# JohnLCaron/electionguard-remote

Hardware: AMD Instinct MI355X
Metric: ballots verified+tallied/sec (node, 4096-bit group) (higher is better)
Workload: dtype u32xu32->u64 (radix-2^29 limbs)

## Files before the change

electionguard-remote_amd/csrc/eg_capi.hip:

```cpp
#include <hip/hip_runtime.h>

#include <algorithm>
#pragma clang diagnostic ignored "-Wunused-result"
#pragma clang diagnostic ignored "-Wunused-value"
#include <cstdio>
#include <cstdlib>
#include <cstring>
#include <deque>
#include <functional>
#include <array>
#include <atomic>
#include <chrono>
#include <condition_variable>
#include <map>
#include <memory>
#include <mutex>
#include <thread>
#include <string>
#include <vector>

#include "../../include/eg_hip.h"
#include "../../include/eg_hip_manifest.h"
#include "../../include/eg_hip_codes.h"
#include "../../include/eg_hip_contestdata.h"
// ... 113 lines not shown
  W_IN0, W_IN1, W_EXP, W_OUT, W_E0, W_E1, W_E2, W_E3, W_JOBS, W_SCR, W_TMP, W_FLAGS, W_SCAL,
  W_BE0, W_BE1, W_BE2, W_OK0, W_OK1, W_OFF, W_H0, W_H1, W_H2, W_H3, W_H4, W_H5, W_H6, W_H7, W_H8, W_EB0, W_EB1, W_EB2, W_EA2, W_YA, W_YB, W_RZ, W_CRF, W_CAST, W_ANY, W_GATHER, W_KBE, W_STAGE, W_NSLOT
};

struct eg_ctx {
  int device = 0;
  hipStream_t stream = nullptr;
  std::mutex mu;
  MontConsts h{};
  MontConsts* d = nullptr;
  uint8_t p_be[512], q_be[32], g_be[512];
  uint8_t* d_q = nullptr;
  uint8_t* d_qbar = nullptr;
  eg_fixed_base* gtab = nullptr;
  eg_fixed_base* Ktab = nullptr;
  uint32_t* d_gcomb = nullptr;
  uint32_t hash_fmt = EG_HASH_FIXED_WIDTH;
  uint32_t resp_plus = 0;
  uint32_t pre_order = EG_PREIMAGE_MESSAGE_FIRST;
  DevBuf ws[W_NSLOT];
  bool timing = false;
  std::vector<ProfRec> prof;
  uint64_t* d_clk = nullptr;
  size_t clk_used = 0;
  uint32_t clk_used_last = 0, clk_dropped_last = 0;
  uint8_t K_be[512];
  struct KeyTabs {
    std::array<uint8_t, 512> K;
    eg_fixed_base* fb = nullptr;
    eg_fixed_base* ct = nullptr;
    uint8_t* d_K = nullptr;
  };
  std::vector<KeyTabs> keys;
  std::map<std::string, DevBuf> cache;
  std::map<std::string, SchedBuf> sched;
  uint32_t use_comb = 1;
  uint32_t ct_encrypt = 0;
  uint32_t ct_pow = 0;
  std::atomic<uint32_t> ct_pow_submit{0};
  int ct_window = kCtEncWindow;
  eg_fixed_base* g_ct = nullptr;
  uint32_t ct_rows = 4;
  uint32_t sel_rows = 4;
  uint32_t sel_blocks = 3;
  size_t pow_slots = 0;
  uint32_t pow_wps = 3;
  double prof_clock_ghz = 0;
  std::vector<std::pair<std::array<uint8_t, 512>, eg_fixed_base*>> share_keys;
  std::shared_ptr<struct Coalescer> co;
  std::mutex co_mu;
  bool co_closed = false;
  hipStream_t copy = nullptr;
  hipEvent_t up_ev[2] = {nullptr, nullptr}, done_ev[2] = {nullptr, nullptr};
  void* comm = nullptr;
  int comm_world = 1, comm_rank = 0;
  bool comm_failed = false;
  std::string comm_fail_msg;
  Pow16Consts* lat = nullptr;
  size_t lat_jobs = 0;
  PowWaveConsts* latw = nullptr;
  size_t latw_jobs = 0;
  size_t wave_max = 0;
  bool wave_split = true;
  size_t r2l_max = 0;
  size_t w8_max = 0;
  int co_zc = 2;
  bool fb_lds = false;
  int test_fail_jobs = 0;
};

static int ws_get(eg_ctx* c, Slot s, size_t bytes, void** out) {
  DevBuf& b = c->ws[s];
  if (b.bytes < bytes) {
    if (b.ptr) HIPCHK(hipFree(b.ptr));
    b.ptr = nullptr;
    b.bytes = 0;
    size_t want = std::max(bytes, (size_t)4096);
    hipError_t e = hipMalloc(&b.ptr, want);
    if (e != hipSuccess) return fail(EG_ERR_NOMEM, "hipMalloc workspace " + std::to_string(want) + " B failed");
    b.bytes = want;
  }
  *out = b.ptr;
  return EG_OK;
}

#define LAUNCH_F(c, K, grid, ...)                                                              \
  do {                                                                                        \
    if ((c)->h.friendly)                                                                      \
      hipLaunchKernelGGL(K<true>, grid, dim3(kBlock), 0, (c)->stream, __VA_ARGS__);            \
    else                                                                                      \
      hipLaunchKernelGGL(K<false>, grid, dim3(kBlock), 0, (c)->stream, __VA_ARGS__);           \
  } while (0)

static inline unsigned grid_for(size_t groups) { return (unsigned)((groups + kGroupsPerBlock - 1) / kGroupsPerBlock); }
static inline size_t padded_groups(size_t groups) { return (size_t)grid_for(groups) * kGroupsPerBlock; }
static inline unsigned cgrid(size_t n) { return (unsigned)((n + 255) / 256); }

static bool aligned16(std::initializer_list<const void*> ps) {
  for (const void* p : ps)
    if ((uintptr_t)p & 15) return false;
  return true;
}

struct StreamOps {
  eg_ctx* c;
  int alloc(size_t bytes, void** out) const { return ws_get(c, W_STAGE, bytes, out); }
  int h2d(void* dst, const void* src, size_t bytes) const {
    HIPCHK(hipMemcpyAsync(dst, src, bytes, hipMemcpyHostToDevice, c->stream));
    return EG_OK;
  }
  int d2h(void* dst, const void* src, size_t bytes) const {
    HIPCHK(hipMemcpyAsync(dst, src, bytes, hipMemcpyDeviceToHost, c->stream));
    return EG_OK;
  }
  int sync() const {
    HIPCHK(hipStreamSynchronize(c->stream));
    return EG_OK;
  }
};
struct Stage : egstage::Stage<StreamOps> {
  Stage(eg_ctx* c, bool host, size_t n, size_t chunk) : egstage::Stage<StreamOps>(StreamOps{c}, host, n, chunk) {}
};

static int launch_import(eg_ctx* c, const uint8_t* d_be, size_t n, uint32_t* d_out, uint8_t* d_ltp) {
  if (!n) return EG_OK;
  LAUNCH_F(c, k_import, dim3(grid_for(n)), c->d, d_be, (uint32_t)n, d_out, d_ltp);
  HIPCHK(hipGetLastError());
  return EG_OK;
}
static int launch_export(eg_ctx* c, const uint32_t* d_in, size_t n, uint8_t* d_be) {
  if (!n) return EG_OK;
  LAUNCH_F(c, k_export, dim3(grid_for(n)), c->d, d_in, (uint32_t)n, d_be);
  HIPCHK(hipGetLastError());
  return EG_OK;
}

static std::vector<uint32_t> pow_schedule(const MontConsts& H, const PowShape& S, const FbTab& f0, const FbTab& f1,
                                          MMCount* mm) {
  std::vector<uint32_t> v;
  MMCount n;
  auto op = [&](PowOp k, uint32_t arg = 0) {
    v.push_back(pow_op(k, arg));
    if (k == OP_SQR) n.sqr += 1;
    else if (k != OP_END && k <= kOpMulLast) n.mul += 1;
  };
// ... 203 lines not shown
    uint32_t* scr = scratch;
    if (!scr) {
      const int rc = ws_get(c, W_SCR, padded_groups(nj) * per + padded_groups(nt) * per1 + padded_groups(nt2) * per2,
                            (void**)&scr);
      if (rc) return rc;
    }
    PowPart P0{S, sched, d_jobs + off * kJobWords, (uint32_t)nj, grid_for(nj), scr,
               yout ? yout + off * (kCombH - 1) * kW : nullptr, ygat, rout ? rout + off * 2 * kW : nullptr, ctab};
    PowPart P1{}, P2{};
    if (nt) {
      P1 = PowPart{tail->S, sched_tail, tail->jobs, (uint32_t)nt, grid_for(nt),
                   scr + padded_groups(nj) * per / 4, tail->yout, tail->ygat, tail->rout, tail->ctab};
    }
    if (nt2) {
      P2 = PowPart{tail2->S, sched_tail2, tail2->jobs, (uint32_t)nt2, grid_for(nt2),
                   scr + (padded_groups(nj) * per + padded_groups(nt) * per1) / 4, tail2->yout, tail2->ygat,
                   tail2->rout, tail2->ctab};
    }
    const dim3 grid(P0.nblocks + P1.nblocks + P2.nblocks);
    ProfRec* pr = nullptr;
    uint64_t* clk = nullptr;
    if (c->timing) {
      c->prof.push_back(ProfRec{nullptr, nullptr,
                                (mm_job.mul + mm_job.sqr) * (double)nj + (mm_tail.mul + mm_tail.sqr) * (double)nt +
                                    (mm_tail2.mul + mm_tail2.sqr) * (double)nt2,
                                mm_job.sqr * (double)nj + mm_tail.sqr * (double)nt + mm_tail2.sqr * (double)nt2});
      pr = &c->prof.back();
      HIPCHK(hipEventCreate(&pr->a));
      HIPCHK(hipEventCreate(&pr->b));
      if (c->d_clk && c->clk_used + grid.x <= kClockRecs) {
        clk = c->d_clk + 2 * c->clk_used;
        c->clk_used += grid.x;
      }
      HIPCHK(hipEventRecord(pr->a, c->stream));
    }
    if (c->h.friendly) {
      if (ct) hipLaunchKernelGGL((k_pow<true, true>), grid, dim3(kBlock), 0, c->stream, c->d, P0, P1, P2, d_elems, d_scal, d_out, f0, f1, clk);
      else hipLaunchKernelGGL((k_pow<true, false>), grid, dim3(kBlock), 0, c->stream, c->d, P0, P1, P2, d_elems, d_scal, d_out, f0, f1, clk);
    } else {
      if (ct) hipLaunchKernelGGL((k_pow<false, true>), grid, dim3(kBlock), 0, c->stream, c->d, P0, P1, P2, d_elems, d_scal, d_out, f0, f1, clk);
      else hipLaunchKernelGGL((k_pow<false, false>), grid, dim3(kBlock), 0, c->stream, c->d, P0, P1, P2, d_elems, d_scal, d_out, f0, f1, clk);
    }
    HIPCHK(hipGetLastError());
    if (pr) HIPCHK(hipEventRecord(pr->b, c->stream));
    off += nj;
  } while (off < njobs);
  return EG_OK;
}

template <class Pass>
static int prod_tree(eg_ctx* c, size_t groups, size_t len, size_t stride, uint32_t* d_out, Pass pass) {
  if (!groups) return EG_OK;
  if (len == 0) return fail(EG_ERR_ARG, "empty product");
  const uint32_t chunk = len > 32 ? 8u : 32u;
  const size_t maxpart = groups * ((len + chunk - 1) / chunk);
  uint32_t* tmp = nullptr;
  int rc = ws_get(c, W_TMP, std::max<size_t>(1, maxpart) * kW * 4 * 2, (void**)&tmp);
  if (rc) return rc;
  uint32_t* ping[2] = {tmp, tmp + maxpart * kW};
  size_t cur_len = len, cur_stride = stride;
  const uint32_t* src = nullptr;
  int pi = 0;
  while (true) {
    const uint32_t nchunk = (uint32_t)((cur_len + chunk - 1) / chunk);
    const bool last = nchunk == 1;
    uint32_t* dst = last ? d_out : ping[pi];
    pass(src, (uint32_t)cur_len, (uint32_t)cur_stride, last ? (uint32_t)cur_len : chunk, nchunk, dst, last);
    HIPCHK(hipGetLastError());
    if (last) break;
    src = dst;
    cur_len = nchunk;
    cur_stride = 1;
    pi ^= 1;
  }
  return EG_OK;
}

static int run_prod(eg_ctx* c, const uint32_t* d_in, GroupMap gm, size_t groups, size_t len, size_t stride,
                    uint32_t* d_out, const uint8_t* mask = nullptr) {
  return prod_tree(c, groups, len, stride, d_out,
                   [&](const uint32_t* src, uint32_t n, uint32_t st, uint32_t ch, uint32_t nchunk, uint32_t* dst, bool) {
                     LAUNCH_F(c, k_prod, dim3(grid_for(groups * nchunk)), c->d, src ? src : d_in,
                              src ? GroupMap{1, 1, 0, 0, n} : gm, (uint32_t)groups, n, st, ch, nchunk, dst,
                              src ? nullptr : mask);
                   });
}

static int run_prod_tab(eg_ctx* c, const uint32_t* d_in, const uint32_t* tab, size_t period, size_t period_stride,
                        size_t groups, size_t len, size_t stride, uint32_t* d_out, const uint32_t* otab,
                        size_t ostride, const uint8_t* mask = nullptr) {
  return prod_tree(c, groups, len, stride, d_out,
                   [&](const uint32_t* src, uint32_t n, uint32_t st, uint32_t ch, uint32_t nchunk, uint32_t* dst, bool last) {
                     LAUNCH_F(c, k_prod_tab, dim3(grid_for(groups * nchunk)), c->d, src ? src : d_in,
                              src ? nullptr : tab, (uint32_t)period, src ? n : (uint32_t)period_stride,
                              (uint32_t)groups, n, st, ch, nchunk, dst, last ? otab : nullptr, (uint32_t)ostride,
                              src ? nullptr : mask);
                   });
}

static int build_fb(eg_ctx* c, const uint32_t* d_base_mont, int wbits, eg_fixed_base* fb) {
  const int nwin = (256 + wbits - 1) / wbits;
  const size_t entries = (size_t)nwin << wbits;
  HIPCHK(hipMalloc(&fb->d_tab, entries * kW * 4));
  fb->wbits = wbits;
  fb->nwin = nwin;
  uint32_t* P = nullptr;
  const int npow = nwin * wbits;
  HIPCHK(hipMalloc(&P, (size_t)npow * kW * 4));
  LAUNCH_F(c, k_sqr_chain, dim3(1), c->d, d_base_mont, (uint32_t)npow, P);
  HIPCHK(hipGetLastError());
  for (int k = 0; k < nwin; ++k) {
    uint32_t* row = fb->d_tab + ((size_t)k << wbits) * kW;
    HIPCHK(hipMemcpyAsync(row, c->d->one, kW * 4, hipMemcpyDeviceToDevice, c->stream));
    for (int a = 0; a < wbits; ++a)
      HIPCHK(hipMemcpyAsync(row + ((size_t)1 << a) * kW, P + (size_t)(k * wbits + a) * kW, kW * 4,
                            hipMemcpyDeviceToDevice, c->stream));
  }
  for (int a = 1; a < wbits; ++a) {
    const size_t njobs = (size_t)nwin * (((size_t)1 << a) - 1);
    LAUNCH_F(c, k_fb_level, dim3(grid_for(njobs)), c->d, fb->d_tab,
                       (uint32_t)wbits, (uint32_t)nwin, (uint32_t)a);
    HIPCHK(hipGetLastError());
  }
  HIPCHK(hipStreamSynchronize(c->stream));
  HIPCHK(hipFree(P));
  return EG_OK;
}

static int import_one(eg_ctx* c, const uint8_t be[512], uint32_t** d_mont_out) {
  uint8_t* d_be = nullptr;
  uint32_t* d_m = nullptr;
  HIPCHK(hipMalloc(&d_be, 512));
  HIPCHK(hipMalloc(&d_m, kW * 4));
  HIPCHK(hipMemcpyAsync(d_be, be, 512, hipMemcpyHostToDevice, c->stream));
  int rc = launch_import(c, d_be, 1, d_m, nullptr);
  if (rc) return rc;
  HIPCHK(hipStreamSynchronize(c->stream));
  HIPCHK(hipFree(d_be));
  *d_mont_out = d_m;
  return EG_OK;
}

static int fb_create_locked(eg_ctx* c, const uint8_t base_be[512], int wbits, eg_fixed_base** out) {
  if (wbits < 4 || wbits > 22)
    return fail(EG_ERR_ARG, "window_bits must be in [4, 22]");
  uint32_t* d_m = nullptr;
  int rc = import_one(c, base_be, &d_m);
  if (rc) return rc;
  auto* fb = new eg_fixed_base();
// ... 39 lines not shown
  unit[0] = 1;
  words_to_elem(unit, c->h.unit);
  for (int i = 0; i < 128; ++i) c->h.pw[i] = p[i];
  uint32_t inv = 1;
  for (int i = 0; i < 6; ++i) inv *= 2u - p[0] * inv;
  c->h.n0 = (0u - inv) & kMask;
  c->h.friendly = c->h.n0 == 1 ? 1u : 0u;
  c->h.mask = kMask;
  {
    const char* lp = getenv("EG_LATENCY_POW");
    const std::string mode = lp ? lp : "";
    std::string err;
    if (mode != "0" && pow16_consts_create(p.data(), r2.data(), r.data(), c->h.n0, c->h.friendly, &c->lat, &err) == 0)
      c->lat_jobs = pow16_round_jobs(device) / 2;
    if (mode != "0" && mode != "16" &&
        powwave_consts_create(p.data(), r2.data(), r.data(), c->h.n0, c->h.friendly, &c->latw, &err) == 0) {
      int cus = 0;
      if (hipDeviceGetAttribute(&cus, hipDeviceAttributeMultiprocessorCount, device) == hipSuccess) {
        c->latw_jobs = (size_t)cus * 4;
        c->r2l_max = (size_t)cus;
        c->w8_max = (size_t)cus;
      }
      if (const char* w8 = getenv("EG_WAVE_W8")) c->w8_max = (size_t)std::max(0L, atol(w8));
      if (const char* rl = getenv("EG_WAVE_R2L")) c->r2l_max = (size_t)std::max(0L, atol(rl));
      if (const char* zc = getenv("EG_COALESCE_ZC")) {
        const std::string z = zc;
        c->co_zc = z == "in" ? 1 : z == "out" ? 2 : z == "inout" ? 3 : 0;
      }
      c->wave_max = c->latw_jobs;
      if (const char* wm = getenv("EG_WAVE_MAX")) c->wave_max = (size_t)std::max(0L, atol(wm));
      if (const char* ws = getenv("EG_WAVE_SPLIT")) c->wave_split = ws[0] != '0';
    }
  }
  {
    const Big q = be_to_words(q_be, 32);
    int64_t br = 0;
    for (int i = 0; i < 8; ++i) {
      br += -(int64_t)q[i];
      c->h.qc[i] = (uint32_t)br;
      br >>= 32;
    }
    c->h.qc_bits = 0;
    for (int b = 255; b >= 0; --b)
      if ((c->h.qc[b >> 5] >> (b & 31)) & 1u) { c->h.qc_bits = (uint32_t)b + 1; break; }
  }
  if (const char* nc = getenv("EG_NO_COMB")) c->use_comb = (nc[0] == '1') ? 0u : 1u;
  if (const char* cr = getenv("EG_CT_ROWS")) c->ct_rows = (cr[0] == '5') ? 0u : 4u;
  if (const char* sc = getenv("EG_SEL_COMB")) {
    c->sel_rows = (sc[0] == '5') ? 0u : 4u;
    c->sel_blocks = (sc[0] == '5') ? 2u : (sc[1] == '2' ? 2u : (sc[1] == '4' ? 4u : 3u));
  }
  if (const char* tf = getenv("EG_TEST_FAIL_JOBS")) c->test_fail_jobs = atoi(tf);
  if (const char* fl = getenv("EG_FB_LDS")) c->fb_lds = fl[0] == '1';
  if (const char* cw = getenv("EG_CT_WINDOW")) c->ct_window = std::max(4, std::min((int)kCtMaxWindow, atoi(cw)));
  {
    int cus = 0, per_cu = 0;
    const char* ts = getenv("EG_TAIL_SPLIT");
    if (!(ts && ts[0] == '0') && hipDeviceGetAttribute(&cus, hipDeviceAttributeMultiprocessorCount, device) == hipSuccess &&
        hipOccupancyMaxActiveBlocksPerMultiprocessor(&per_cu, k_pow<true, false>, kBlock, 0) == hipSuccess && per_cu > 0) {
      c->pow_slots = (size_t)cus * (size_t)per_cu;
      c->pow_wps = (uint32_t)std::max(1, per_cu * (kBlock / 64) / 4);
    }
  }
  hipError_t e = hipStreamCreateWithFlags(&c->stream, hipStreamNonBlocking);
  if (e != hipSuccess) {
    delete c;
    return fail(EG_ERR_HIP, std::string("hipStreamCreate: ") + hipGetErrorString(e));
  }
  auto setup = [&]() -> int {
    HIPCHK(hipMalloc(&c->d, sizeof(MontConsts)));
    HIPCHK(hipMemcpy(c->d, &c->h, sizeof(MontConsts), hipMemcpyHostToDevice));
    HIPCHK(hipMalloc(&c->d_q, 32));
    HIPCHK(hipMemcpy(c->d_q, q_be, 32, hipMemcpyHostToDevice));
    HIPCHK(hipMalloc(&c->d_qbar, 32));
    std::lock_guard<std::mutex> lk(c->mu);
    return fb_create_locked(c, g_be, 8, &c->gtab);
  };
  const int rc = setup();
  if (rc) {
    const std::string msg = g_err;
    eg_ctx_destroy(c);
    return fail(rc, msg);
  }
  *out = c;
  return EG_OK;
}

extern "C" int eg_fixed_base_destroy(eg_fixed_base* fb) {
  if (!fb) return EG_OK;
  while (fb->queued.load(std::memory_order_acquire) > 0) std::this_thread::sleep_for(std::chrono::microseconds(20));
  if (fb->d_tab) hipFree(fb->d_tab);
  eg_fixed_base_destroy(fb->ct);
  delete fb;
  return EG_OK;
}

static int ct_table_locked(eg_ctx* c, eg_fixed_base* fb, FbTab* out) {
  if (fb->wbits <= (int)kCtMaxWindow) {
    *out = fb->tab();
    return EG_OK;
  }
  if (!fb->ct) {
    const int rc = fb_create_locked(c, fb->base.data(), kCtEncWindow, &fb->ct);
    if (rc) return rc;
  }
  *out = fb->ct->tab();
  return EG_OK;
}

static void coalescer_stop(eg_ctx* c);
static int comm_destroy_locked(eg_ctx* c);

extern "C" int eg_ctx_destroy(eg_ctx* c) {
  if (!c) return EG_OK;
  coalescer_stop(c);
  hipSetDevice(c->device);
  hipStreamSynchronize(c->stream);
  comm_destroy_locked(c);
  eg_fixed_base_destroy(c->gtab);
  for (auto& k : c->keys) {
    eg_fixed_base_destroy(k.fb);
    eg_fixed_base_destroy(k.ct);
    if (k.d_K) hipFree(k.d_K);
  }
  eg_fixed_base_destroy(c->g_ct);
  for (auto& kv : c->share_keys) eg_fixed_base_destroy(kv.second);
  for (auto& b : c->ws)
    if (b.ptr) hipFree(b.ptr);
  for (auto& kv : c->cache)
    if (kv.second.ptr) hipFree(kv.second.ptr);
  for (auto& kv : c->sched) hipFree(const_cast<uint32_t*>(kv.second.ptr));
  for (auto& r : c->prof) {
    if (r.a) hipEventDestroy(r.a);
    if (r.b) hipEventDestroy(r.b);
  }
  if (c->d_clk) hipFree(c->d_clk);
  pow16_consts_destroy(c->lat);
  powwave_consts_destroy(c->latw);
  if (c->d) hipFree(c->d);
  if (c->d_q) hipFree(c->d_q);
  if (c->d_qbar) hipFree(c->d_qbar);
  if (c->d_gcomb) hipFree(c->d_gcomb);
  if (c->copy) {
    hipStreamSynchronize(c->copy);
    hipStreamDestroy(c->copy);
  }
  for (int i = 0; i < 2; ++i) {
    if (c->up_ev[i]) hipEventDestroy(c->up_ev[i]);
    if (c->done_ev[i]) hipEventDestroy(c->done_ev[i]);
  }
  if (c->stream) hipStreamDestroy(c->stream);
  delete c;
  return EG_OK;
}

extern "C" int eg_ctx_sync(eg_ctx* c) {
  if (!c) return fail(EG_ERR_ARG, "null ctx");
  HIPCHK(hipSetDevice(c->device));
  HIPCHK(hipStreamSynchronize(c->stream));
  return EG_OK;
}

extern "C" eg_fixed_base* eg_ctx_g_table(eg_ctx* c) { return c ? c->gtab : nullptr; }

extern "C" int eg_ctx_set_hash_format(eg_ctx* c, int format) {
  if (!c) return fail(EG_ERR_ARG, "null ctx");
  if (format != EG_HASH_FIXED_WIDTH && format != EG_HASH_MINIMAL) return fail(EG_ERR_ARG, "unknown hash format");
  std::lock_guard<std::mutex> lk(c->mu);
  c->hash_fmt = (uint32_t)format;
  return EG_OK;
}

extern "C" int eg_ctx_set_proof_format(eg_ctx* c, int response, int preimage) {
  if (!c) return fail(EG_ERR_ARG, "null ctx");
  if (response != EG_RESPONSE_MINUS && response != EG_RESPONSE_PLUS) return fail(EG_ERR_ARG, "unknown response convention");
  if (preimage < EG_PREIMAGE_MESSAGE_FIRST || preimage > EG_PREIMAGE_WITH_KEY)
    return fail(EG_ERR_ARG, "unknown pre-image order");
  std::lock_guard<std::mutex> lk(c->mu);
  c->resp_plus = response == EG_RESPONSE_PLUS ? 1u : 0u;
  c->pre_order = (uint32_t)preimage;
  return EG_OK;
}

extern "C" int eg_fixed_base_create(eg_ctx* c, const uint8_t base_be[512], int wbits, eg_fixed_base** out) {
  if (!c || !base_be || !out) return fail(EG_ERR_ARG, "null argument");
  std::lock_guard<std::mutex> lk(c->mu);
  HIPCHK(hipSetDevice(c->device));
  return fb_create_locked(c, base_be, wbits, out);
}

struct Locked {
  std::lock_guard<std::mutex> lk;
  explicit Locked(eg_ctx* c) : lk(c->mu) { hipSetDevice(c->device); }
};

static int upload(eg_ctx* c, Slot s, const void* h, size_t bytes, void** d) {
  int rc = ws_get(c, s, bytes, d);
  if (rc) return rc;
  HIPCHK(hipMemcpyAsync(*d, h, bytes, hipMemcpyHostToDevice, c->stream));
// ... 356 lines not shown
```

electionguard-remote_amd/csrc/eg_capi_ballot.inc:

```

static int upload_job_table(eg_ctx* c, const std::vector<uint32_t>& host, DevBuf* out) {
  DevBuf b;
  b.bytes = std::max<size_t>(4, host.size() * 4);
  if (c->test_fail_jobs > 0 && --c->test_fail_jobs == 0)
    return fail(EG_ERR_NOMEM, "hipMalloc job table failed (EG_TEST_FAIL_JOBS)");
  if (hipMalloc(&b.ptr, b.bytes) != hipSuccess)
    return fail(EG_ERR_NOMEM, "hipMalloc job table " + std::to_string(b.bytes) + " B failed");
  const hipError_t e = hipMemcpy(b.ptr, host.data(), host.size() * 4, hipMemcpyHostToDevice);
  if (e != hipSuccess) {
    hipFree(b.ptr);
    return fail(EG_ERR_HIP, std::string("hipMemcpy job table: ") + hipGetErrorString(e));
  }
  *out = b;
  return EG_OK;
}

static int cache_bound(eg_ctx* c) {
  if (c->cache.size() < 64) return EG_OK;
  HIPCHK(hipStreamSynchronize(c->stream));
  for (auto& kv : c->cache) HIPCHK(hipFree(kv.second.ptr));
  c->cache.clear();
  return EG_OK;
}

// ... 235 lines not shown
    std::vector<uint32_t> t;
    for (uint32_t k : C.members)
      for (uint32_t comp = 0; comp < 2; ++comp) t.push_back(M.first[k] * 2 + comp);
    return t;
  });
  L.add("out" + C.tag, &T.out[ci], [&C]() {
    std::vector<uint32_t> t;
    for (uint32_t k : C.members)
      for (uint32_t comp = 0; comp < 2; ++comp) t.push_back(k * 2 + comp);
    return t;
  });
}

static int contest_aggregates(eg_ctx* c, const ManShape& M, const ContestTabs& T, size_t nbc, const uint32_t* elems,
                              uint32_t* agg) {
  if (M.uniform)
    return run_prod(c, elems, GroupMap{2, (uint32_t)M.nc, 1, 2 * M.uspc, (uint32_t)(2 * M.nsel)}, nbc * M.nc * 2,
                    M.uspc, 2, agg);
  for (size_t ci = 0; ci < M.cls.size(); ++ci) {
    const size_t period = M.cls[ci].n * 2;
    const int rc = run_prod_tab(c, elems, T.in[ci], period, 2 * M.nsel, nbc * period, M.cls[ci].spc, 2, agg,
                                T.out[ci], 2 * M.nc);
    if (rc) return rc;
  }
  return EG_OK;
}
static void contest_scalars(eg_ctx* c, const ManShape& M, const ContestTabs& T, uint8_t* sc, size_t ncn, uint8_t* negL,
                            uint8_t* okc) {
  if (M.uniform)
    hipLaunchKernelGGL(k_scalar_prep, dim3(cgrid(ncn)), dim3(256), 0, c->stream, c->d_q, sc, (uint32_t)ncn, 2u, 0u,
                       M.ulimit, negL, okc, c->resp_plus, 0x1u);
  else
    hipLaunchKernelGGL(k_scalar_prep_tab, dim3(cgrid(ncn)), dim3(256), 0, c->stream, c->d_q, sc, (uint32_t)ncn, 2u, 0u,
                       T.limit, (uint32_t)M.nc, negL, okc, c->resp_plus, 0x1u);
}
static void contest_flags(eg_ctx* c, const ManShape& M, const ContestTabs& T, const uint8_t* ltp, size_t ncn,
                          uint8_t* crf) {
  if (M.uniform)
    hipLaunchKernelGGL(k_contest_flags, dim3(cgrid(ncn * 2)), dim3(256), 0, c->stream, ltp, (uint32_t)ncn, M.uspc,
                       crf);
  else
    hipLaunchKernelGGL(k_contest_flags_seg, dim3(cgrid(ncn * 2)), dim3(256), 0, c->stream, ltp, (uint32_t)ncn,
                       (uint32_t)M.nc, (uint32_t)M.nsel, T.first, T.spc, crf);
}
static void nonce_sums(eg_ctx* c, const ManShape& M, const ContestTabs& T, const uint8_t* sc, size_t ncn,
                       uint8_t* rsum) {
  if (M.uniform)
    hipLaunchKernelGGL(k_enc_rsum, dim3(cgrid(ncn)), dim3(256), 0, c->stream, c->d_q, sc, (uint32_t)ncn, M.uspc, rsum);
  else
    hipLaunchKernelGGL(k_enc_rsum_seg, dim3(cgrid(ncn)), dim3(256), 0, c->stream, c->d_q, sc, (uint32_t)ncn,
                       (uint32_t)M.nc, (uint32_t)M.nsel, T.first, T.spc, rsum);
}
static int chunk_tally(eg_ctx* c, const ManShape& M, const ContestTabs& T, size_t nbc, const uint32_t* elems,
                       uint32_t* out, const uint8_t* d_cast) {
  if (M.uniform)
    return run_prod(c, elems, GroupMap{2, M.uspc - M.uph, 1, 2, 2 * M.uspc}, M.nreal * 2, nbc, M.nsel * 2, out, d_cast);
  return run_prod_tab(c, elems, T.tally, M.nreal * 2, 0, M.nreal * 2, nbc, M.nsel * 2, out, nullptr, 0, d_cast);
}

struct VerifyLayout {
  size_t ns, ncn, off_c, off_neg, off_negL;
  VerifyLayout(const ManShape& M, size_t nbc)
      : ns(nbc * M.nsel), ncn(nbc * M.nc), off_c(ns * 4), off_neg(off_c + ncn * 2), off_negL(off_neg + ns) {}
};
static std::vector<uint32_t> verify_sel_jobs(const VerifyLayout& V, bool beta) {
  auto J = new_jobs(V.ns);
  for (size_t i = 0; i < V.ns; ++i) {
    uint32_t* x = &J[i * kJobWords];
    const uint32_t c0 = (uint32_t)(i * 4), v0 = c0 + 1, c1 = c0 + 2, v1 = c0 + 3, e = beta ? 1u : 0u;
    x[0] = (uint32_t)(i * 2) + e; x[1] = c0; x[2] = c1; x[3] = c0 + e; x[4] = c1 + e; x[5] = v0; x[7] = v1;
    if (beta) x[8] = (uint32_t)(V.off_neg + i);
  }
  return J;
}
static std::vector<uint32_t> verify_contest_jobs(const ManShape& M, const ManShape::Class& C, const VerifyLayout& V,
                                                 size_t nbc, bool b) {
  auto J = new_jobs(nbc * C.n);
  for (size_t bi = 0; bi < nbc; ++bi)
    for (size_t mi = 0; mi < C.n; ++mi) {
      const uint32_t k = M.member(C, mi), e = b ? 1u : 0u;
      const size_t j = bi * M.nc + k;
      uint32_t* x = &J[(bi * C.n + mi) * kJobWords];
      const uint32_t cc = (uint32_t)(V.off_c + j * 2);
      x[0] = (uint32_t)(V.ns * 2 + j * 2) + e; x[1] = cc; x[3] = (uint32_t)(V.ns * 4 + j * 2) + e; x[5] = cc + 1;
      if (b) x[6] = (uint32_t)(V.off_negL + j);
      x[2] = (uint32_t)(bi * M.nsel + M.first_of(k));
    }
  return J;
}

struct Pop {
  PowShape S;
  const uint32_t* jobs;
  size_t n;
  const uint32_t* ygat;
  Pop part(size_t off, size_t cnt) const { return Pop{S, jobs + off * kJobWords, cnt, ygat}; }
  PowTail tail() const {
    PowTail T{};
    T.S = S; T.jobs = jobs; T.njobs = n; T.ygat = ygat;
    return T;
  }
};
struct PowLaunch {
  Pop main;
  std::vector<Pop> tails;
};
struct VerifyPlan {
  size_t xb = 0;
  std::vector<Pop> l2;
  std::vector<PowLaunch> later;
// ... 103 lines not shown
    if ((rc = ws_get(c, W_YA, ns * (kCombH - 1) * kW * 4, (void**)&YA))) return rc;
    if ((rc = ws_get(c, W_YB, ns * (kCombH - 1) * kW * 4, (void**)&YB))) return rc;
  }
  if ((rc = ws_get(c, W_RZ, ns * 4 * kW * 4, (void**)&RZ))) return rc;
  const uint32_t srows = c->sel_rows, sblocks = c->sel_blocks;
  PowShape SA{};
  SA.has_base = 1; SA.nout = 2; SA.nfb[0] = 1; SA.nfb[1] = 1; SA.exp_bytes = 32; SA.comb = 1; SA.resid = 1;
  SA.rows = srows; SA.blocks = sblocks; SA.tab[0][0] = 0; SA.tab[1][0] = 0;
  PowShape SB{};
  SB.has_base = 1; SB.nout = 2; SB.nfb[0] = 1; SB.nfb[1] = 2; SB.exp_bytes = 32; SB.comb = 1; SB.resid = 1;
  SB.rows = srows; SB.blocks = sblocks; SB.tab[0][0] = 1; SB.tab[1][0] = 1; SB.tab[1][1] = 0;
  std::vector<Pop> pa, pb;
  for (size_t ci = 0; ci < ncls; ++ci) {
    const uint32_t gather = gat ? M.cls[ci].spc : 0u;
    const size_t n = nbc * M.cls[ci].n;
    PowShape SCA{};
    SCA.has_base = 1; SCA.nout = 1; SCA.nfb[0] = 1; SCA.exp_bytes = 32; SCA.tab[0][0] = 0;
    SCA.comb = gat ? 1u : 0u; SCA.gather = gather;
    PowShape SCB{};
    SCB.has_base = 1; SCB.nout = 1; SCB.nfb[0] = 2; SCB.exp_bytes = 32; SCB.tab[0][0] = 1; SCB.tab[0][1] = 0;
    SCB.comb = gat ? 1u : 0u; SCB.gather = gather;
    pa.push_back(Pop{SCA, jCA[ci], n, YA});
    pb.push_back(Pop{SCB, jCB[ci], n, YB});
  }
  const VerifyPlan P = plan_pow_launches(c, M, ns, ncn, pa, pb);
  const size_t xb = P.xb;
  auto launch = [&](const PowShape& S, const uint32_t* jobs, size_t n, uint32_t* yout, const uint32_t* ygat,
                    uint32_t* rout, const std::vector<PowTail>& tl) {
    return launch_pow(c, S, jobs, n, E, SC, COMM, G, K, yout, ygat, tl.size() > 0 ? &tl[0] : nullptr, rout, false,
                      nullptr, nullptr, tl.size() > 1 ? &tl[1] : nullptr);
  };
  auto tails_of = [](const std::vector<Pop>& pops) {
    std::vector<PowTail> tl;
    for (const Pop& p : pops) tl.push_back(p.tail());
    return tl;
  };
  {
    PowTail H{};
    H.S = SB; H.jobs = jB; H.njobs = xb; H.yout = YB; H.rout = RZ + ns * 2 * kW;
    if ((rc = launch(SA, jA, ns, YA, nullptr, RZ, {H}))) return rc;
  }
  if ((rc = launch(SB, jB + xb * kJobWords, ns - xb, gat ? YB + xb * (kCombH - 1) * kW : nullptr, nullptr,
                   RZ + (ns + xb) * 2 * kW, tails_of(P.l2))))
    return rc;
  LAUNCH_F(c, k_resid_check, dim3(grid_for(ns)), c->d, RZ, (uint32_t)ns, LTP, 2u);
  LAUNCH_F(c, k_resid_check, dim3(grid_for(ns)), c->d, RZ + ns * 2 * kW, (uint32_t)ns, LTP + 1, 2u);
  HIPCHK(hipGetLastError());
  uint8_t* CRF = nullptr;
  if ((rc = ws_get(c, W_CRF, ncn * 2, (void**)&CRF))) return rc;
  contest_flags(c, M, T, LTP, ncn, CRF);
  HIPCHK(hipGetLastError());
  for (const PowLaunch& l : P.later)
    if ((rc = launch(l.main.S, l.main.jobs, l.main.n, nullptr, l.main.ygat, nullptr, tails_of(l.tails)))) return rc;
  if ((rc = launch_export(c, COMM, ns * 4 + ncn * 2, COMM_BE))) return rc;
  if ((rc = launch_export(c, CP, ncn * 2, CP_BE))) return rc;
  if ((rc = launch_hash(c, (uint32_t)ns,
                        preimage(c, {HashSrc{cts, 512, 1024}, HashSrc{cts + 512, 512, 1024}},
                                 {HashSrc{COMM_BE, 512, 2048}, HashSrc{COMM_BE + 512, 512, 2048},
                                  HashSrc{COMM_BE + 1024, 512, 2048}, HashSrc{COMM_BE + 1536, 512, 2048}},
                                 key_src(c)),
                        d_rproof, 4, 0, 2, OKR, LTP, 2, d_ok_sel, nullptr)))
    return rc;
  const uint8_t* CC_BE = COMM_BE + ns * 4 * 512;
  if ((rc = launch_hash(c, (uint32_t)ncn,
                        preimage(c, {HashSrc{CP_BE, 512, 1024}, HashSrc{CP_BE + 512, 512, 1024}},
                                 {HashSrc{CC_BE, 512, 1024}, HashSrc{CC_BE + 512, 512, 1024}}, key_src(c)),
                        d_cproof, 2, 0, kNone, OKC, CRF, 2, d_ok_con, nullptr)))
    return rc;
  if (tally) {
    uint32_t* TP = first ? tally : tally + nreal * 2 * kW;
    if ((rc = chunk_tally(c, M, T, nbc, E, TP, d_cast))) return rc;
    if (!first) {
      LAUNCH_F(c, k_mul, dim3(grid_for(nreal * 2)), c->d, tally, 1u, TP, 1u, (uint32_t)(nreal * 2), tally, 1u);
      HIPCHK(hipGetLastError());
    }
  }
  return EG_OK;
}

static int use_key_locked(eg_ctx* c, const uint8_t* K_be) {
  for (size_t i = 0; i < c->keys.size(); ++i)
    if (std::memcmp(c->keys[i].K.data(), K_be, 512) == 0) {
      key_front(c, i);
      return EG_OK;
    }
  const int wb = c->Ktab ? c->Ktab->wbits : c->gtab->wbits;
  return set_key_locked(c, K_be, wb, false);
}

static void ones_be(uint8_t* out, size_t n) {
  std::memset(out, 0, n * 512);
  for (size_t i = 0; i < n; ++i) out[i * 512 + 511] = 1;
}

static int verify_dev_locked(eg_ctx* c, const ManShape& M, const uint8_t* qbar_be, size_t nb, const uint8_t* d_cts,
                             const uint8_t* d_rproof, const uint8_t* d_cproof, const uint8_t* d_cast,
                             uint8_t* d_ok_sel, uint8_t* d_ok_con, uint8_t* d_tally_be) {
  int rc;
  const size_t nc = M.nc, nsel = M.nsel, nreal = M.nreal;
  if (!nb) {
    if (d_tally_be) {
      std::vector<uint8_t> one(nreal * 2 * 512);
      ones_be(one.data(), nreal * 2);
      HIPCHK(hipMemcpyAsync(d_tally_be, one.data(), one.size(), hipMemcpyHostToDevice, c->stream));
      HIPCHK(hipStreamSynchronize(c->stream));
    }
    return EG_OK;
  }
  if (!c->Ktab) return fail(EG_ERR_STATE, "election key not set (eg_set_election_key)");
  HIPCHK(hipMemcpyAsync(c->d_qbar, qbar_be, 32, hipMemcpyHostToDevice, c->stream));
  uint32_t* tally = nullptr;
  if (d_tally_be && (rc = ws_get(c, W_E2, nreal * 2 * 2 * kW * 4, (void**)&tally))) return rc;
  const size_t chunk = ballot_chunk(nsel);
  for (size_t b0 = 0; b0 < nb; b0 += chunk) {
    const size_t nbc = std::min(chunk, nb - b0);
    if ((rc = verify_chunk_locked(c, M, nbc, d_cts + b0 * nsel * 1024, d_rproof + b0 * nsel * 128,
                                  d_cproof + b0 * nc * 64, d_cast ? d_cast + b0 : nullptr, d_ok_sel + b0 * nsel,
                                  d_ok_con + b0 * nc, tally, b0 == 0)))
      return rc;
  }
  return d_tally_be ? launch_export(c, tally, nreal * 2, d_tally_be) : EG_OK;
}

static int ensure_copy_stream(eg_ctx* c) {
  if (c->copy) return EG_OK;
  HIPCHK(hipStreamCreateWithFlags(&c->copy, hipStreamNonBlocking));
  for (int i = 0; i < 2; ++i) {
    HIPCHK(hipEventCreateWithFlags(&c->up_ev[i], hipEventDisableTiming));
// ... 537 lines not shown
```

electionguard-remote_amd/csrc/eg_kernels.hpp:

```cpp
#pragma once
#include "eg_bignum.hpp"
#include "eg_sha256.hpp"

namespace eg {

constexpr int kBlock = 256;
#ifndef EG_SQR
#define EG_SQR 1
#endif
#ifndef EG_MASK_RT
#define EG_MASK_RT 2
#endif
#ifndef EG_TRAFFIC_X2
#define EG_TRAFFIC_X2 0
#endif
#ifndef EG_MIN_WAVES
#define EG_MIN_WAVES 3
#endif
constexpr int kGroupsPerBlock = kBlock / kT;
constexpr uint32_t kNone = 0xFFFFFFFFu;

struct FbTab {
  const uint32_t* data;
  uint32_t wbits;
// ... 17 lines not shown
#else
    const uint32_t* s = C->p + glane() * kLP;
#pragma unroll
    for (int j = 0; j < kL; ++j) p[j] = s[j];
#endif
    n0 = C->n0;
#if EG_MASK_RT == 2
    mask = kMask;
    asm volatile("" : "+v"(mask));
#elif EG_MASK_RT
    mask = C->mask;
#else
    mask = kMask;
#endif
  }
  __device__ __forceinline__ void mul(uint32_t (&x)[kL], const uint32_t* y) const {
    mont_mul_impl<F, false>(x, y, p, n0, mask);
  }
  __device__ __forceinline__ void redc(uint32_t (&x)[kL]) const { mont_redc_impl<F>(x, p, n0, mask); }
  __device__ __forceinline__ void sqr(uint32_t (&x)[kL], const uint32_t* y) const {
#if EG_SQR
    mont_mul_impl<F, true>(x, y, p, n0, mask);
#else
    mont_mul_impl<F, false>(x, y, p, n0, mask);
#endif
  }
};

__device__ __forceinline__ uint32_t* group_slot() {
  __shared__ uint32_t s_slots[kGroupsPerBlock * kYStride];
  return s_slots + (threadIdx.x / kT) * kYStride;
}
__device__ __forceinline__ uint32_t group_id() { return blockIdx.x * kGroupsPerBlock + threadIdx.x / kT; }

__device__ __forceinline__ void wave_sync() { __builtin_amdgcn_wave_barrier(); }

template <bool F>
__device__ __forceinline__ void msqr(const Mont<F>& M, uint32_t (&x)[kL], uint32_t* slot) {
  regs_to_lds(slot, x);
  wave_sync();
  M.sqr(x, slot);
  wave_sync();
}
template <bool F>
__device__ __forceinline__ void mmul_g(const Mont<F>& M, uint32_t (&x)[kL], uint32_t* slot,
                                       const uint32_t* __restrict__ E) {
  elem_to_lds(slot, E);
  wave_sync();
  M.mul(x, slot);
  wave_sync();
}


__device__ __forceinline__ void stage_be(uint32_t* slot, const uint8_t* __restrict__ be) {
  constexpr int kPer = 32 / kT;
  const uint4* src = reinterpret_cast<const uint4*>(be);
#pragma unroll
  for (int k = 0; k < kPer; ++k) {
    const int idx = glane() * kPer + k;
    const uint4 v = src[idx];
    slot[127 - 4 * idx] = __builtin_bswap32(v.x);
    slot[126 - 4 * idx] = __builtin_bswap32(v.y);
    slot[125 - 4 * idx] = __builtin_bswap32(v.z);
    slot[124 - 4 * idx] = __builtin_bswap32(v.w);
  }
}

template <bool F>
__global__ void __launch_bounds__(kBlock) k_import(const MontConsts* __restrict__ C,
                                                   const uint8_t* __restrict__ be, uint32_t n,
                                                   uint32_t* __restrict__ out, uint8_t* __restrict__ lt_p) {
  const uint32_t gid = group_id();
  const uint32_t e = gid < n ? gid : n - 1;
  uint32_t* slot = group_slot();
  Mont<F> M;
  M.load(C);
  stage_be(slot, be + (size_t)e * 512);
  wave_sync();
  uint32_t x[kL];
#pragma unroll
  for (int j = 0; j < kL; ++j) x[j] = bits_limb(slot, kLimbBits * (glane() * kL + j));
  if (lt_p != nullptr) {
    constexpr int kWords = 128 / kT;
    int cmp = 0;
#pragma unroll
    for (int i = kWords - 1; i >= 0; --i) {
      const int w = glane() * kWords + i;
      const uint32_t a = slot[w], b = C->pw[w];
      if (cmp == 0) cmp = a < b ? -1 : (a > b ? 1 : 0);
    }
    const uint32_t sh = gslot() * kT;
    const uint32_t lt = (uint32_t)(__ballot(cmp < 0) >> sh) & ((1u << kT) - 1u);
    const uint32_t ne = (uint32_t)(__ballot(cmp != 0) >> sh) & ((1u << kT) - 1u);
    if (glane() == 0 && gid < n) lt_p[gid] = ne ? (uint8_t)((lt >> (31 - __builtin_clz(ne))) & 1u) : 0;
  }
  wave_sync();
  elem_to_lds(slot, C->r2);
  wave_sync();
  M.mul(x, slot);
  if (gid < n) store_elem(out + (size_t)gid * kW, x);
}

template <bool F>
__device__ __forceinline__ void regs_normalize(const Mont<F>& M, uint32_t (&x)[kL]) {
  uint32_t c = 0;
#pragma unroll
  for (int j = 0; j < kL; ++j) {
    const uint32_t v = x[j] + c;
    x[j] = v & kMask;
    c = v >> kLimbBits;
  }
  const bool g0 = glane() == 0;
  for (int round = 0; round < kT; ++round) {
    uint32_t cin = from_prev(c);
    if (g0) cin = 0;
    if (__ballot(cin != 0) == 0) break;
    c = 0;
    if (cin) {
#pragma unroll
      for (int j = 0; j < kL; ++j) {
        const uint32_t v = x[j] + cin;
        x[j] = v & kMask;
        cin = v >> kLimbBits;
      }
      c = cin;
    }
  }
  bool eq = true;
#pragma unroll
  for (int j = 0; j < kL; ++j) eq &= x[j] == M.p[j];
  const uint64_t gmask = (uint64_t)((1u << kT) - 1u) << (gslot() * kT);
  if ((__ballot(!eq) & gmask) == 0) {
#pragma unroll
    for (int j = 0; j < kL; ++j) x[j] = 0;
  }
}

__device__ __forceinline__ void slot_to_be(uint32_t* slot, uint8_t* __restrict__ dst, bool do_store) {
  constexpr int kPer = 128 / kT;
#pragma unroll
  for (int k = 0; k < kPer; ++k) {
    const int b = glane() * kPer + k;
    const int w = 127 - b;
    const int bit = 32 * w;
    const int a = bit / kLimbBits, sh = bit - a * kLimbBits;
    auto limb = [&](int i) -> uint64_t {
      return i < kN ? (uint64_t)slot[(i / kL) * kLP + (i % kL)] : 0ull;
    };
    const uint64_t v = (limb(a) >> sh) | (limb(a + 1) << (kLimbBits - sh)) |
                       (limb(a + 2) << (2 * kLimbBits - sh));
    if (do_store) reinterpret_cast<uint32_t*>(dst)[b] = __builtin_bswap32((uint32_t)v);
  }
}

template <bool F>
__global__ void __launch_bounds__(kBlock) k_export(const MontConsts* __restrict__ C,
                                                   const uint32_t* __restrict__ in, uint32_t n,
                                                   uint8_t* __restrict__ be) {
  const uint32_t gid = group_id();
  const uint32_t e = gid < n ? gid : n - 1;
  uint32_t* slot = group_slot();
  Mont<F> M;
  M.load(C);
  uint32_t x[kL];
  load_elem(x, in + (size_t)e * kW);
  M.redc(x);
  regs_normalize(M, x);
  regs_to_lds(slot, x);
  wave_sync();
  slot_to_be(slot, be + (size_t)gid * 512, gid < n);
}

template <bool F>
__device__ __forceinline__ void regs_reduce_lazy(const Mont<F>& M, uint32_t (&x)[kL]) {
  uint32_t c = 0;
#pragma unroll
  for (int j = 0; j < kL; ++j) {
    const uint32_t v = x[j] + c;
    x[j] = v & kMask;
    c = v >> kLimbBits;
  }
  const bool g0 = glane() == 0;
  for (int round = 0; round < kT; ++round) {
    uint32_t cin = from_prev(c);
    if (g0) cin = 0;
    if (__ballot(cin != 0) == 0) break;
    c = 0;
    if (cin) {
#pragma unroll
      for (int j = 0; j < kL; ++j) {
        const uint32_t v = x[j] + cin;
        x[j] = v & kMask;
        cin = v >> kLimbBits;
      }
      c = cin;
    }
  }
  bool ne = false, gt = false;
#pragma unroll
  for (int j = 0; j < kL; ++j) {
    if (x[j] != M.p[j]) { ne = true; gt = x[j] > M.p[j]; }
  }
  const uint32_t sh = gslot() * kT;
  const uint32_t nem = (uint32_t)(__ballot(ne) >> sh) & ((1u << kT) - 1u);
  const uint32_t gtm = (uint32_t)(__ballot(gt) >> sh) & ((1u << kT) - 1u);
  const bool ge = nem == 0 || ((gtm >> (31 - __builtin_clz(nem))) & 1u);
  if (__ballot(ge) == 0) return;
  uint32_t b = 0;
  if (ge) {
#pragma unroll
    for (int j = 0; j < kL; ++j) {
      const uint32_t v = x[j] - M.p[j] - b;
      x[j] = v & kMask;
      b = v >> 31;
    }
  }
  for (int round = 0; round < kT; ++round) {
    uint32_t bin = from_prev(b);
    if (g0) bin = 0;
    if (__ballot(bin != 0) == 0) break;
    b = 0;
    if (bin) {
#pragma unroll
// ... 781 lines not shown
```

Baseline: 34260.

## Overlap tally on side stream, adapt product-tree fan-in, vectorize import/export conversion

Tally product-tree kernels now run on a separate non-blocking stream, so they can overlap with export and hashing of the verify batch, joined through events. The product tree chooses its fan-in per level from how well the level fills the GPU, dropping to 2 when work is small. Import and export replace per-limb bit extraction and the LDS-staged r2 with coalesced uint4 byte swaps, alignbit word-to-limb conversion, a register-based less-than-p check, and r2 held in shared memory. These changes add stream and event management, a block barrier in import, and more intricate bit-packing code that could contain edge-case errors.

```diff
diff --git a/electionguard-remote_amd/csrc/eg_capi.hip b/electionguard-remote_amd/csrc/eg_capi.hip
--- a/electionguard-remote_amd/csrc/eg_capi.hip
+++ b/electionguard-remote_amd/csrc/eg_capi.hip
@@ -189,6 +189,9 @@
   bool co_closed = false;
   hipStream_t copy = nullptr;
   hipEvent_t up_ev[2] = {nullptr, nullptr}, done_ev[2] = {nullptr, nullptr};
+  hipStream_t side = nullptr;
+  hipEvent_t side_go = nullptr, side_done = nullptr;
+  bool tally_side = true;
   void* comm = nullptr;
   int comm_world = 1, comm_rank = 0;
   bool comm_failed = false;
@@ -221,13 +224,14 @@
   return EG_OK;
 }
 
-#define LAUNCH_F(c, K, grid, ...)                                                              \
+#define LAUNCH_FS(c, s, K, grid, ...)                                                          \
   do {                                                                                        \
     if ((c)->h.friendly)                                                                      \
-      hipLaunchKernelGGL(K<true>, grid, dim3(kBlock), 0, (c)->stream, __VA_ARGS__);            \
+      hipLaunchKernelGGL(K<true>, grid, dim3(kBlock), 0, s, __VA_ARGS__);                      \
     else                                                                                      \
-      hipLaunchKernelGGL(K<false>, grid, dim3(kBlock), 0, (c)->stream, __VA_ARGS__);           \
+      hipLaunchKernelGGL(K<false>, grid, dim3(kBlock), 0, s, __VA_ARGS__);                     \
   } while (0)
+#define LAUNCH_F(c, K, grid, ...) LAUNCH_FS(c, (c)->stream, K, grid, __VA_ARGS__)
 
 static inline unsigned grid_for(size_t groups) { return (unsigned)((groups + kGroupsPerBlock - 1) / kGroupsPerBlock); }
 static inline size_t padded_groups(size_t groups) { return (size_t)grid_for(groups) * kGroupsPerBlock; }
@@ -537,8 +541,13 @@
 static int prod_tree(eg_ctx* c, size_t groups, size_t len, size_t stride, uint32_t* d_out, Pass pass) {
   if (!groups) return EG_OK;
   if (len == 0) return fail(EG_ERR_ARG, "empty product");
-  const uint32_t chunk = len > 32 ? 8u : 32u;
-  const size_t maxpart = groups * ((len + chunk - 1) / chunk);
+  const size_t fill = std::max<size_t>(1, c->pow_slots ? c->pow_slots / c->pow_wps : 256) * kGroupsPerBlock;
+  auto fan_of = [&](size_t n, bool first) -> uint32_t {
+    if (first && n <= 32) return 32u;
+    return groups * ((n + 7) / 8) >= fill ? 8u : 2u;
+  };
+  const uint32_t fan0 = fan_of(len, true);
+  const size_t maxpart = groups * ((len + fan0 - 1) / fan0);
   uint32_t* tmp = nullptr;
   int rc = ws_get(c, W_TMP, std::max<size_t>(1, maxpart) * kW * 4 * 2, (void**)&tmp);
   if (rc) return rc;
@@ -547,6 +556,7 @@
   const uint32_t* src = nullptr;
   int pi = 0;
   while (true) {
+    const uint32_t chunk = fan_of(cur_len, src == nullptr);
     const uint32_t nchunk = (uint32_t)((cur_len + chunk - 1) / chunk);
     const bool last = nchunk == 1;
     uint32_t* dst = last ? d_out : ping[pi];
@@ -562,24 +572,26 @@
 }
 
 static int run_prod(eg_ctx* c, const uint32_t* d_in, GroupMap gm, size_t groups, size_t len, size_t stride,
-                    uint32_t* d_out, const uint8_t* mask = nullptr) {
+                    uint32_t* d_out, const uint8_t* mask = nullptr, hipStream_t s = nullptr) {
+  if (!s) s = c->stream;
   return prod_tree(c, groups, len, stride, d_out,
                    [&](const uint32_t* src, uint32_t n, uint32_t st, uint32_t ch, uint32_t nchunk, uint32_t* dst, bool) {
-                     LAUNCH_F(c, k_prod, dim3(grid_for(groups * nchunk)), c->d, src ? src : d_in,
-                              src ? GroupMap{1, 1, 0, 0, n} : gm, (uint32_t)groups, n, st, ch, nchunk, dst,
-                              src ? nullptr : mask);
+                     LAUNCH_FS(c, s, k_prod, dim3(grid_for(groups * nchunk)), c->d, src ? src : d_in,
+                               src ? GroupMap{1, 1, 0, 0, n} : gm, (uint32_t)groups, n, st, ch, nchunk, dst,
+                               src ? nullptr : mask);
                    });
 }
 
 static int run_prod_tab(eg_ctx* c, const uint32_t* d_in, const uint32_t* tab, size_t period, size_t period_stride,
                         size_t groups, size_t len, size_t stride, uint32_t* d_out, const uint32_t* otab,
-                        size_t ostride, const uint8_t* mask = nullptr) {
+                        size_t ostride, const uint8_t* mask = nullptr, hipStream_t s = nullptr) {
+  if (!s) s = c->stream;
   return prod_tree(c, groups, len, stride, d_out,
                    [&](const uint32_t* src, uint32_t n, uint32_t st, uint32_t ch, uint32_t nchunk, uint32_t* dst, bool last) {
-                     LAUNCH_F(c, k_prod_tab, dim3(grid_for(groups * nchunk)), c->d, src ? src : d_in,
-                              src ? nullptr : tab, (uint32_t)period, src ? n : (uint32_t)period_stride,
-                              (uint32_t)groups, n, st, ch, nchunk, dst, last ? otab : nullptr, (uint32_t)ostride,
-                              src ? nullptr : mask);
+                     LAUNCH_FS(c, s, k_prod_tab, dim3(grid_for(groups * nchunk)), c->d, src ? src : d_in,
+                               src ? nullptr : tab, (uint32_t)period, src ? n : (uint32_t)period_stride,
+                               (uint32_t)groups, n, st, ch, nchunk, dst, last ? otab : nullptr, (uint32_t)ostride,
+                               src ? nullptr : mask);
                    });
 }
 
@@ -725,6 +737,7 @@
   }
   if (const char* tf = getenv("EG_TEST_FAIL_JOBS")) c->test_fail_jobs = atoi(tf);
   if (const char* fl = getenv("EG_FB_LDS")) c->fb_lds = fl[0] == '1';
+  if (const char* tsd = getenv("EG_TALLY_STREAM")) c->tally_side = tsd[0] != '0';
   if (const char* cw = getenv("EG_CT_WINDOW")) c->ct_window = std::max(4, std::min((int)kCtMaxWindow, atoi(cw)));
   {
     int cus = 0, per_cu = 0;
@@ -818,6 +831,12 @@
     hipStreamSynchronize(c->copy);
     hipStreamDestroy(c->copy);
   }
+  if (c->side) {
+    hipStreamSynchronize(c->side);
+    hipStreamDestroy(c->side);
+  }
+  if (c->side_go) hipEventDestroy(c->side_go);
+  if (c->side_done) hipEventDestroy(c->side_done);
   for (int i = 0; i < 2; ++i) {
     if (c->up_ev[i]) hipEventDestroy(c->up_ev[i]);
     if (c->done_ev[i]) hipEventDestroy(c->done_ev[i]);
diff --git a/electionguard-remote_amd/csrc/eg_capi_ballot.inc b/electionguard-remote_amd/csrc/eg_capi_ballot.inc
--- a/electionguard-remote_amd/csrc/eg_capi_ballot.inc
+++ b/electionguard-remote_amd/csrc/eg_capi_ballot.inc
@@ -311,10 +311,18 @@
                        (uint32_t)M.nc, (uint32_t)M.nsel, T.first, T.spc, rsum);
 }
 static int chunk_tally(eg_ctx* c, const ManShape& M, const ContestTabs& T, size_t nbc, const uint32_t* elems,
-                       uint32_t* out, const uint8_t* d_cast) {
+                       uint32_t* out, const uint8_t* d_cast, hipStream_t s) {
   if (M.uniform)
-    return run_prod(c, elems, GroupMap{2, M.uspc - M.uph, 1, 2, 2 * M.uspc}, M.nreal * 2, nbc, M.nsel * 2, out, d_cast);
-  return run_prod_tab(c, elems, T.tally, M.nreal * 2, 0, M.nreal * 2, nbc, M.nsel * 2, out, nullptr, 0, d_cast);
+    return run_prod(c, elems, GroupMap{2, M.uspc - M.uph, 1, 2, 2 * M.uspc}, M.nreal * 2, nbc, M.nsel * 2, out, d_cast,
+                    s);
+  return run_prod_tab(c, elems, T.tally, M.nreal * 2, 0, M.nreal * 2, nbc, M.nsel * 2, out, nullptr, 0, d_cast, s);
+}
+static int ensure_side_stream(eg_ctx* c) {
+  if (c->side) return EG_OK;
+  HIPCHK(hipStreamCreateWithFlags(&c->side, hipStreamNonBlocking));
+  HIPCHK(hipEventCreateWithFlags(&c->side_go, hipEventDisableTiming));
+  HIPCHK(hipEventCreateWithFlags(&c->side_done, hipEventDisableTiming));
+  return EG_OK;
 }
 
 struct VerifyLayout {
@@ -524,6 +532,11 @@
   HIPCHK(hipGetLastError());
   for (const PowLaunch& l : P.later)
     if ((rc = launch(l.main.S, l.main.jobs, l.main.n, nullptr, l.main.ygat, nullptr, tails_of(l.tails)))) return rc;
+  const bool side = tally && c->tally_side;
+  if (side) {
+    if ((rc = ensure_side_stream(c))) return rc;
+    HIPCHK(hipEventRecord(c->side_go, c->stream));
+  }
   if ((rc = launch_export(c, COMM, ns * 4 + ncn * 2, COMM_BE))) return rc;
   if ((rc = launch_export(c, CP, ncn * 2, CP_BE))) return rc;
   if ((rc = launch_hash(c, (uint32_t)ns,
@@ -540,12 +553,19 @@
                         d_cproof, 2, 0, kNone, OKC, CRF, 2, d_ok_con, nullptr)))
     return rc;
   if (tally) {
+    const hipStream_t ts = side ? c->side : c->stream;
+    if (side) HIPCHK(hipStreamWaitEvent(ts, c->side_go, 0));
     uint32_t* TP = first ? tally : tally + nreal * 2 * kW;
-    if ((rc = chunk_tally(c, M, T, nbc, E, TP, d_cast))) return rc;
-    if (!first) {
-      LAUNCH_F(c, k_mul, dim3(grid_for(nreal * 2)), c->d, tally, 1u, TP, 1u, (uint32_t)(nreal * 2), tally, 1u);
-      HIPCHK(hipGetLastError());
-    }
+    rc = chunk_tally(c, M, T, nbc, E, TP, d_cast, ts);
+    if (!rc && !first) {
+      LAUNCH_FS(c, ts, k_mul, dim3(grid_for(nreal * 2)), c->d, tally, 1u, TP, 1u, (uint32_t)(nreal * 2), tally, 1u);
+      if (hipGetLastError() != hipSuccess) rc = fail(EG_ERR_HIP, "k_mul launch failed");
+    }
+    if (side) {
+      HIPCHK(hipEventRecord(c->side_done, ts));
+      HIPCHK(hipStreamWaitEvent(c->stream, c->side_done, 0));
+    }
+    if (rc) return rc;
   }
   return EG_OK;
 }
diff --git a/electionguard-remote_amd/csrc/eg_kernels.hpp b/electionguard-remote_amd/csrc/eg_kernels.hpp
--- a/electionguard-remote_amd/csrc/eg_kernels.hpp
+++ b/electionguard-remote_amd/csrc/eg_kernels.hpp
@@ -93,17 +93,39 @@
 }
 
 
+constexpr int kLaneBits = kL * kLimbBits;
+constexpr int kLaneWords = (kLaneBits + 31) / 32;
+static_assert(kLaneBits % 32 != 0, "a lane's first bit must share a word with the lane below (words_to_slot)");
+static_assert((kT - 1) * kLaneBits / 32 + kLaneWords + 1 <= kYStride, "the top lane's window stays inside the slot");
+__device__ __forceinline__ uint32_t lane_bit0() { return (uint32_t)glane() * kLaneBits; }
+
 __device__ __forceinline__ void stage_be(uint32_t* slot, const uint8_t* __restrict__ be) {
   constexpr int kPer = 32 / kT;
   const uint4* src = reinterpret_cast<const uint4*>(be);
 #pragma unroll
   for (int k = 0; k < kPer; ++k) {
-    const int idx = glane() * kPer + k;
+    const int idx = k * kT + glane();
     const uint4 v = src[idx];
-    slot[127 - 4 * idx] = __builtin_bswap32(v.x);
-    slot[126 - 4 * idx] = __builtin_bswap32(v.y);
-    slot[125 - 4 * idx] = __builtin_bswap32(v.z);
-    slot[124 - 4 * idx] = __builtin_bswap32(v.w);
+    *reinterpret_cast<uint4*>(slot + 124 - 4 * idx) =
+        make_uint4(__builtin_bswap32(v.w), __builtin_bswap32(v.z), __builtin_bswap32(v.y), __builtin_bswap32(v.x));
+  }
+  if (glane() == 0) *reinterpret_cast<uint4*>(slot + 128) = make_uint4(0u, 0u, 0u, 0u);
+}
+
+__device__ __forceinline__ void slot_words_to_limbs(uint32_t (&x)[kL], const uint32_t* slot) {
+  const uint32_t b0 = lane_bit0(), s0 = b0 & 31u;
+  const uint32_t* w = slot + (b0 >> 5);
+  uint32_t r[kLaneWords + 1], a[kLaneWords];
+#pragma unroll
+  for (int i = 0; i <= kLaneWords; ++i) r[i] = w[i];
+#pragma unroll
+  for (int i = 0; i < kLaneWords; ++i) a[i] = __builtin_amdgcn_alignbit(r[i + 1], r[i], s0);
+#pragma unroll
+  for (int j = 0; j < kL; ++j) {
+    const int i = (j * kLimbBits) >> 5, sh = (j * kLimbBits) & 31;
+    uint32_t v = a[i] >> sh;
+    if (sh + kLimbBits > 32) v |= a[i + 1 < kLaneWords ? i + 1 : i] << ((32 - sh) & 31);
+    x[j] = v & kMask;
   }
 }
 
@@ -111,34 +133,33 @@
 __global__ void __launch_bounds__(kBlock) k_import(const MontConsts* __restrict__ C,
                                                    const uint8_t* __restrict__ be, uint32_t n,
                                                    uint32_t* __restrict__ out, uint8_t* __restrict__ lt_p) {
+  __shared__ uint32_t s_r2[kW];
+  for (int i = threadIdx.x; i < kW; i += blockDim.x) s_r2[i] = C->r2[i];
   const uint32_t gid = group_id();
   const uint32_t e = gid < n ? gid : n - 1;
   uint32_t* slot = group_slot();
   Mont<F> M;
   M.load(C);
+#if !EG_PLDS
+  __syncthreads();
+#endif
   stage_be(slot, be + (size_t)e * 512);
   wave_sync();
   uint32_t x[kL];
-#pragma unroll
-  for (int j = 0; j < kL; ++j) x[j] = bits_limb(slot, kLimbBits * (glane() * kL + j));
+  slot_words_to_limbs(x, slot);
   if (lt_p != nullptr) {
-    constexpr int kWords = 128 / kT;
-    int cmp = 0;
-#pragma unroll
-    for (int i = kWords - 1; i >= 0; --i) {
-      const int w = glane() * kWords + i;
-      const uint32_t a = slot[w], b = C->pw[w];
-      if (cmp == 0) cmp = a < b ? -1 : (a > b ? 1 : 0);
+    bool ne = false, lt = false;
+#pragma unroll
+    for (int j = 0; j < kL; ++j) {
+      const uint32_t pj = M.p[j];
+      if (x[j] != pj) { ne = true; lt = x[j] < pj; }
     }
     const uint32_t sh = gslot() * kT;
-    const uint32_t lt = (uint32_t)(__ballot(cmp < 0) >> sh) & ((1u << kT) - 1u);
-    const uint32_t ne = (uint32_t)(__ballot(cmp != 0) >> sh) & ((1u << kT) - 1u);
-    if (glane() == 0 && gid < n) lt_p[gid] = ne ? (uint8_t)((lt >> (31 - __builtin_clz(ne))) & 1u) : 0;
-  }
-  wave_sync();
-  elem_to_lds(slot, C->r2);
-  wave_sync();
-  M.mul(x, slot);
+    const uint32_t ltm = (uint32_t)(__ballot(lt) >> sh) & ((1u << kT) - 1u);
+    const uint32_t nem = (uint32_t)(__ballot(ne) >> sh) & ((1u << kT) - 1u);
+    if (glane() == 0 && gid < n) lt_p[gid] = nem ? (uint8_t)((ltm >> (31 - __builtin_clz(nem))) & 1u) : 0;
+  }
+  M.mul(x, s_r2);
   if (gid < n) store_elem(out + (size_t)gid * kW, x);
 }
 
@@ -177,20 +198,50 @@
   }
 }
 
-__device__ __forceinline__ void slot_to_be(uint32_t* slot, uint8_t* __restrict__ dst, bool do_store) {
-  constexpr int kPer = 128 / kT;
-#pragma unroll
-  for (int k = 0; k < kPer; ++k) {
-    const int b = glane() * kPer + k;
-    const int w = 127 - b;
-    const int bit = 32 * w;
-    const int a = bit / kLimbBits, sh = bit - a * kLimbBits;
-    auto limb = [&](int i) -> uint64_t {
-      return i < kN ? (uint64_t)slot[(i / kL) * kLP + (i % kL)] : 0ull;
-    };
-    const uint64_t v = (limb(a) >> sh) | (limb(a + 1) << (kLimbBits - sh)) |
-                       (limb(a + 2) << (2 * kLimbBits - sh));
-    if (do_store) reinterpret_cast<uint32_t*>(dst)[b] = __builtin_bswap32((uint32_t)v);
+__device__ __forceinline__ void limbs_to_slot_words(uint32_t* slot, const uint32_t (&x)[kL]) {
+  uint32_t a[kLaneWords + 1];
+#pragma unroll
+  for (int i = 0; i <= kLaneWords; ++i) a[i] = 0;
+#pragma unroll
+  for (int j = 0; j < kL; ++j) {
+    const int i = (j * kLimbBits) >> 5, sh = (j * kLimbBits) & 31;
+    a[i] |= x[j] << sh;
+    if (sh + kLimbBits > 32) a[i + 1] |= x[j] >> ((32 - sh) & 31);
+  }
+  const uint32_t b0 = lane_bit0(), s0 = b0 & 31u;
+  uint32_t b[kLaneWords + 1];
+  b[0] = a[0] << s0;
+#pragma unroll
+  for (int i = 1; i <= kLaneWords; ++i) b[i] = (uint32_t)(((((uint64_t)a[i]) << 32) | a[i - 1]) >> (32u - s0));
+  const uint32_t top = (s0 + kLaneBits) >> 5;
+  uint32_t above = from_next(b[0]);
+  if (glane() == kT - 1) above = 0;
+  uint32_t* w = slot + (b0 >> 5);
+  if (glane() == 0) w[0] = b[0];
+#pragma unroll
+  for (int i = 1; i < kLaneWords - 1; ++i) w[i] = b[i];
+  w[kLaneWords - 1] = b[kLaneWords - 1] | (top == kLaneWords - 1 ? above : 0u);
+  if (top == kLaneWords) w[kLaneWords] = b[kLaneWords] | above;
+}
+
+__device__ __forceinline__ void slot_words_to_be(const uint32_t* slot, uint8_t* __restrict__ dst, bool do_store) {
+  if (((uintptr_t)dst & 15u) == 0) {
+    constexpr int kPer = 32 / kT;
+#pragma unroll
+    for (int k = 0; k < kPer; ++k) {
+      const int idx = k * kT + glane();
+      const uint4 v = *reinterpret_cast<const uint4*>(slot + 124 - 4 * idx);
+      if (do_store)
+        reinterpret_cast<uint4*>(dst)[idx] = make_uint4(__builtin_bswap32(v.w), __builtin_bswap32(v.z),
+                                                        __builtin_bswap32(v.y), __builtin_bswap32(v.x));
+    }
+  } else {
+    constexpr int kPer = 128 / kT;
+#pragma unroll
+    for (int k = 0; k < kPer; ++k) {
+      const int bw = k * kT + glane();
+      if (do_store) reinterpret_cast<uint32_t*>(dst)[bw] = __builtin_bswap32(slot[127 - bw]);
+    }
   }
 }
 
@@ -207,9 +258,9 @@
   load_elem(x, in + (size_t)e * kW);
   M.redc(x);
   regs_normalize(M, x);
-  regs_to_lds(slot, x);
+  limbs_to_slot_words(slot, x);
   wave_sync();
-  slot_to_be(slot, be + (size_t)gid * 512, gid < n);
+  slot_words_to_be(slot, be + (size_t)gid * 512, gid < n);
 }
 
 template <bool F>
```

Result: no change. 34320 (median of 6 runs) (+0.2%).
